# lxa9867/ImageFolder

Hardware: NVIDIA H100
Metric: tokenizer_train_images_per_sec_256x256 (higher is better)
Workload: dtype bf16

## Files before the change

imagefolder_b200/csrc/attn_kernel.cu:

```cuda
#include "xq_common.cuh"
#include "xq_tc.cuh"

namespace xq {
using namespace xqtc;

constexpr int AT_BM = 128;
constexpr int AT_BN = 128;
constexpr int AT_D = 64;
constexpr int AT_NS = 2;
constexpr int AT_TILE = AT_BM * AT_D * 2;
constexpr int AT_THREADS = 288;

struct AttnFwdSmem {
    static constexpr int Q = 0;
    static constexpr int K = AT_TILE;
    static constexpr int V = AT_TILE * (1 + AT_NS);
    static constexpr int BAR = AT_TILE * (1 + 2 * AT_NS);
    static constexpr int BYTES = BAR + 256;
};

__device__ __forceinline__ void named_bar_sync(int id, int nthreads) { asm volatile("bar.sync %0, %1;" ::"r"(id), "r"(nthreads) : "memory"); }

__global__ void __launch_bounds__(AT_THREADS, 1)
attn_fwd_kernel(const __grid_constant__ CUtensorMap tmQKV, __nv_bfloat16 *__restrict__ out, float *__restrict__ lse2, int N, int H,
                int nQ , float c ) {
    extern __shared__ uint8_t smem_raw[];
    uint8_t *base = (uint8_t *)(((uintptr_t)smem_raw + 1023) & ~(uintptr_t)1023);
    uint64_t *bars = (uint64_t *)(base + AttnFwdSmem::BAR);
    uint64_t *q_full = bars + 0;
    uint64_t *k_full = bars + 1;
    uint64_t *k_empty = bars + 1 + AT_NS;
    uint64_t *v_full = bars + 1 + 2 * AT_NS;
    uint64_t *v_empty = bars + 1 + 3 * AT_NS;

    const int tid = threadIdx.x, warp = tid >> 5, lane = tid & 31;
    const int nK = (N + AT_BN - 1) / AT_BN;
    const int bh = blockIdx.x / nQ, qt = blockIdx.x - bh * nQ;
    const int b = bh / H, h = bh - b * H;

    if (tid == 0) {
        mbar_init(q_full, 1);
        for (int i = 0; i < AT_NS; ++i) { mbar_init(&k_full[i], 1); mbar_init(&k_empty[i], 8); mbar_init(&v_full[i], 1); mbar_init(&v_empty[i], 8); }
        mbar_fence_init();
    }
    __syncthreads();

    if (warp == 8) {
        const int colQ = h * AT_D, colK = (H + h) * AT_D, colV = (2 * H + h) * AT_D;
        if (elect_one()) {
            tma_prefetch_desc(&tmQKV);
            mbar_expect_tx(q_full, AT_TILE);
            tma_load_3d(base + AttnFwdSmem::Q, &tmQKV, colQ, qt * AT_BM, b, q_full);
        }
        __syncwarp();
        for (int j = 0; j < nK; ++j) {
            const int st = j % AT_NS;
            const uint32_t ph = ((j / AT_NS) & 1) ^ 1;
            mbar_wait(&k_empty[st], ph);
            if (elect_one()) {
                mbar_expect_tx(&k_full[st], AT_TILE);
                tma_load_3d(base + AttnFwdSmem::K + st * AT_TILE, &tmQKV, colK, j * AT_BN, b, &k_full[st]);
            }
            __syncwarp();
            mbar_wait(&v_empty[st], ph);
            if (elect_one()) {
                mbar_expect_tx(&v_full[st], AT_TILE);
                tma_load_3d(base + AttnFwdSmem::V + st * AT_TILE, &tmQKV, colV, j * AT_BN, b, &v_full[st]);
            }
            __syncwarp();
        }
        return;
    }

    const int wg = warp >> 2, wq = warp & 3;
    const int rq = wg * 64 + wq * 16 + (lane >> 2), cq = 2 * (lane & 3);
    const uint64_t qd = desc_k_sw128(smem_u32(base + AttnFwdSmem::Q + wg * (AT_TILE / 2)));
    float m[2] = {-CUDART_INF_F, -CUDART_INF_F}, l[2] = {0.f, 0.f};
    float o[32];
#pragma unroll
    for (int i = 0; i < 32; ++i) o[i] = 0.f;
    mbar_wait(q_full, 0);
    for (int j = 0; j < nK; ++j) {
        const int st = j % AT_NS;
        const uint32_t ph = (j / AT_NS) & 1;
        float s[64];
        mbar_wait(&k_full[st], ph);
        const uint64_t kd = desc_k_sw128(smem_u32(base + AttnFwdSmem::K + st * AT_TILE));
        wgmma_fence();
#pragma unroll
        for (int k = 0; k < AT_D / 16; ++k) wgmma_m64n128k16_ss<0, 0>(s, desc_adv(qd, k * 32), desc_adv(kd, k * 32), (uint32_t)k);
        wgmma_commit();
        wgmma_wait<0>();
        fence_regs(s);
        __syncwarp();
        if (lane == 0) mbar_arrive(&k_empty[st]);
        const int nv = N - j * AT_BN;
        if (nv < AT_BN) {
#pragma unroll
            for (int i = 0; i < 64; ++i)
                if (8 * (i >> 2) + cq + (i & 1) >= nv) s[i] = -CUDART_INF_F;
        }
        float mx[2] = {m[0], m[1]};
#pragma unroll
        for (int i = 0; i < 64; ++i) mx[(i >> 1) & 1] = fmaxf(mx[(i >> 1) & 1], s[i]);
#pragma unroll
        for (int hh = 0; hh < 2; ++hh) {
            mx[hh] = fmaxf(mx[hh], __shfl_xor_sync(0xffffffffu, mx[hh], 1));
            mx[hh] = fmaxf(mx[hh], __shfl_xor_sync(0xffffffffu, mx[hh], 2));
        }
        float alpha[2], mc[2];
#pragma unroll
        for (int hh = 0; hh < 2; ++hh) {
            alpha[hh] = ex2_approx((m[hh] - mx[hh]) * c);
            m[hh] = mx[hh];
            mc[hh] = mx[hh] * c;
            l[hh] *= alpha[hh];
        }
#pragma unroll
        for (int i = 0; i < 32; ++i) o[i] *= alpha[(i >> 1) & 1];
        uint32_t pa[AT_BN / 16][4];
#pragma unroll
        for (int i = 0; i < 64; i += 2) {
            const int hh = (i >> 1) & 1;
            const float p0 = ex2_approx(fmaf(s[i], c, -mc[hh])), p1 = ex2_approx(fmaf(s[i + 1], c, -mc[hh]));
            l[hh] += p0 + p1;
            pa[i >> 3][((i >> 2) & 1) * 2 + hh] = pack_bf16(p0, p1);
        }
        mbar_wait(&v_full[st], ph);
        const uint64_t vd = desc_mn_sw128(smem_u32(base + AttnFwdSmem::V + st * AT_TILE), AT_TILE);
        wgmma_fence();
#pragma unroll
        for (int k = 0; k < AT_BN / 16; ++k) wgmma_m64n64k16_rs<1>(o, pa[k], desc_adv(vd, k * 2048), 1u);
        wgmma_commit();
        wgmma_wait<0>();
        fence_regs(o);
        __syncwarp();
        if (lane == 0) mbar_arrive(&v_empty[st]);
    }
#pragma unroll
    for (int hh = 0; hh < 2; ++hh) {
        l[hh] += __shfl_xor_sync(0xffffffffu, l[hh], 1);
        l[hh] += __shfl_xor_sync(0xffffffffu, l[hh], 2);
    }
#pragma unroll
    for (int hh = 0; hh < 2; ++hh) {
        const int n = qt * AT_BM + rq + 8 * hh;
        if (n >= N) continue;
        const float inv = 1.0f / l[hh];
        if (cq == 0) lse2[(size_t)bh * N + n] = fmaf(m[hh], c, log2f(l[hh]));
        __nv_bfloat16 *orow = out + ((size_t)b * N + n) * H * AT_D + h * AT_D;
#pragma unroll
        for (int jj = 0; jj < AT_D / 8; ++jj)
            *reinterpret_cast<uint32_t *>(orow + 8 * jj + cq) = pack_bf16(o[4 * jj + 2 * hh] * inv, o[4 * jj + 2 * hh + 1] * inv);
    }
}

constexpr int AT_TAIL_MAX = 0;

__global__ void __launch_bounds__(128)
attn_fwd_tail_kernel(const __nv_bfloat16 *__restrict__ qkv, __nv_bfloat16 *__restrict__ out, float *__restrict__ lse2, int B, int N,
                     int H, int n0 , float c) {
    const int lane = threadIdx.x & 31;
    const long long w = ((long long)blockIdx.x * blockDim.x + threadIdx.x) >> 5;
    const int nt = N - n0;
    if (w >= (long long)B * H * nt) return;
    const int r = (int)(w % nt);
    const int bh = (int)(w / nt);
    const int b = bh / H, h = bh - b * H;
    const int n = n0 + r;
    const size_t W = (size_t)3 * H * AT_D;
    const __nv_bfloat16 *qp = qkv + ((size_t)b * N + n) * W + h * AT_D;
    float qf[AT_D];
#pragma unroll
    for (int u = 0; u < 8; ++u) {
        const uint4 x = *reinterpret_cast<const uint4 *>(qp + u * 8);
        const __nv_bfloat162 *x2 = reinterpret_cast<const __nv_bfloat162 *>(&x);
#pragma unroll
        for (int e = 0; e < 4; ++e) {
            const float2 f = __bfloat1622float2(x2[e]);
            qf[u * 8 + 2 * e] = f.x * c;
            qf[u * 8 + 2 * e + 1] = f.y * c;
        }
    }
    float m = -CUDART_INF_F, l = 0.f, o[AT_D];
#pragma unroll
    for (int i = 0; i < AT_D; ++i) o[i] = 0.f;
    for (int key = lane; key < N; key += 32) {
        const __nv_bfloat16 *kp = qkv + ((size_t)b * N + key) * W + (H + h) * AT_D;
        const __nv_bfloat16 *vp = kp + (size_t)H * AT_D;
        float s = 0.f;
#pragma unroll
        for (int u = 0; u < 8; ++u) {
            const uint4 x = *reinterpret_cast<const uint4 *>(kp + u * 8);
            const __nv_bfloat162 *x2 = reinterpret_cast<const __nv_bfloat162 *>(&x);
#pragma unroll
            for (int e = 0; e < 4; ++e) {
                const float2 f = __bfloat1622float2(x2[e]);
                s = fmaf(qf[u * 8 + 2 * e], f.x, s);
                s = fmaf(qf[u * 8 + 2 * e + 1], f.y, s);
            }
        }
        const float m_new = fmaxf(m, s);
        const float corr = ex2_approx(m - m_new);
        const float p = ex2_approx(s - m_new);
        l = fmaf(l, corr, p);
        m = m_new;
#pragma unroll
        for (int u = 0; u < 8; ++u) {
            const uint4 x = *reinterpret_cast<const uint4 *>(vp + u * 8);
            const __nv_bfloat162 *x2 = reinterpret_cast<const __nv_bfloat162 *>(&x);
#pragma unroll
            for (int e = 0; e < 4; ++e) {
                const float2 f = __bfloat1622float2(x2[e]);
                o[u * 8 + 2 * e] = fmaf(o[u * 8 + 2 * e], corr, p * f.x);
                o[u * 8 + 2 * e + 1] = fmaf(o[u * 8 + 2 * e + 1], corr, p * f.y);
            }
        }
    }
    float M = m;
#pragma unroll
    for (int off = 16; off > 0; off >>= 1) M = fmaxf(M, __shfl_xor_sync(0xffffffffu, M, off));
    const float f = (m == -CUDART_INF_F) ? 0.f : ex2_approx(m - M);
    l *= f;
#pragma unroll
    for (int off = 16; off > 0; off >>= 1) l += __shfl_xor_sync(0xffffffffu, l, off);
    const float inv = 1.0f / l;
    float mine0 = 0.f, mine1 = 0.f;
#pragma unroll
    for (int i = 0; i < AT_D; ++i) {
        float x = o[i] * f;
#pragma unroll
        for (int off = 16; off > 0; off >>= 1) x += __shfl_xor_sync(0xffffffffu, x, off);
        if (i == 2 * lane) mine0 = x;
        if (i == 2 * lane + 1) mine1 = x;
    }
    __nv_bfloat16 *op = out + ((size_t)b * N + n) * H * AT_D + h * AT_D;
    *reinterpret_cast<uint32_t *>(op + 2 * lane) = pack_bf16(mine0 * inv, mine1 * inv);
    if (lane == 0) lse2[(size_t)bh * N + n] = M + log2f(l);
}

constexpr int AB_THREADS = 288;
constexpr int AB_BQ = 64;
constexpr int AB_QS = 3;
constexpr int AB_QTILE = AB_BQ * AT_D * 2;

struct AttnBwdSmem {
    static constexpr int K = 0;
    static constexpr int V = AT_TILE;
    static constexpr int Q = 2 * AT_TILE;
    static constexpr int DO = Q + AB_QS * AB_QTILE;
    static constexpr int DS = DO + AB_QS * AB_QTILE;
    static constexpr int STAT = DS + 2 * AB_QTILE;
    static constexpr int BAR = STAT + AB_QS * 512;
    static constexpr int BYTES = BAR + 256;
};

__device__ __forceinline__ void bwd_epilogue_frag(const float (&acc)[32], float mul, __nv_bfloat16 *__restrict__ row0,
                                                  size_t row_stride, bool ok0, bool ok1, float *__restrict__ g_bias_cols, int lane) {
    const int cq = 2 * (lane & 3);
#pragma unroll
    for (int jj = 0; jj < AT_D / 8; ++jj) {
        const uint32_t w0 = pack_bf16(acc[4 * jj] * mul, acc[4 * jj + 1] * mul);
        const uint32_t w1 = pack_bf16(acc[4 * jj + 2] * mul, acc[4 * jj + 3] * mul);
        if (ok0) *reinterpret_cast<uint32_t *>(row0 + 8 * jj + cq) = w0;
        if (ok1) *reinterpret_cast<uint32_t *>(row0 + 8 * row_stride + 8 * jj + cq) = w1;
        if (g_bias_cols) {
            float s0 = __uint_as_float(w0 << 16) + __uint_as_float(w1 << 16);
            float s1 = __uint_as_float(w0 & 0xffff0000u) + __uint_as_float(w1 & 0xffff0000u);
#pragma unroll
            for (int o = 4; o < 32; o <<= 1) {
                s0 += __shfl_xor_sync(0xffffffffu, s0, o);
                s1 += __shfl_xor_sync(0xffffffffu, s1, o);
            }
            if (lane < 4) {
                atomicAdd(g_bias_cols + 8 * jj + cq, s0);
                atomicAdd(g_bias_cols + 8 * jj + cq + 1, s1);
            }
        }
    }
}

__global__ void __launch_bounds__(AB_THREADS, 1)
attn_bwd_kernel(const __grid_constant__ CUtensorMap tmQKV, const __grid_constant__ CUtensorMap tmDO, const float *__restrict__ lseP,
                const float *__restrict__ deltaP, float *__restrict__ dq_acc, __nv_bfloat16 *__restrict__ dqkv, float *__restrict__ g_bias,
                int N, int H, int Npad, float c, float scale) {
    extern __shared__ uint8_t smem_raw[];
    uint8_t *base = (uint8_t *)(((uintptr_t)smem_raw + 1023) & ~(uintptr_t)1023);
    uint64_t *bars = (uint64_t *)(base + AttnBwdSmem::BAR);
    uint64_t *kv_full = bars;
    uint64_t *q_full = bars + 1;
    uint64_t *q_empty = bars + 1 + AB_QS;
    float *s_lse = (float *)(base + AttnBwdSmem::STAT);
    float *s_delta = s_lse + AB_QS * AB_BQ;

    const int tid = threadIdx.x, warp = tid >> 5, lane = tid & 31;
    const int bh = blockIdx.y, b = bh / H, h = bh - b * H;
    const int k0 = blockIdx.x * AT_BN;
    const int colQ = h * AT_D, colK = (H + h) * AT_D, colV = (2 * H + h) * AT_D;
    const int nQ = (N + AB_BQ - 1) / AB_BQ;

    if (tid == 0) {
        mbar_init(kv_full, 1);
        for (int i = 0; i < AB_QS; ++i) { mbar_init(&q_full[i], 1); mbar_init(&q_empty[i], 8); }
        mbar_fence_init();
    }
    __syncthreads();

    if (warp == 8) {
        if (elect_one()) {
            tma_prefetch_desc(&tmQKV);
            tma_prefetch_desc(&tmDO);
            mbar_expect_tx(kv_full, 2 * AT_TILE);
            for (int hf = 0; hf < 2; ++hf) {
                tma_load_3d(base + AttnBwdSmem::K + hf * AB_QTILE, &tmQKV, colK, k0 + hf * AB_BQ, b, kv_full);
                tma_load_3d(base + AttnBwdSmem::V + hf * AB_QTILE, &tmQKV, colV, k0 + hf * AB_BQ, b, kv_full);
            }
        }
        __syncwarp();
        for (int i = 0; i < nQ; ++i) {
            const int st = i % AB_QS;
            mbar_wait(&q_empty[st], ((i / AB_QS) & 1) ^ 1);
// ... 323 lines not shown

static int attn_bwd_ktail(int N) {
    const int r = N % AT_BN;
    return (N > AT_BN && r != 0 && r <= AB_KTAIL_MAX) ? r : 0;
}

static size_t attn_bwd_ws_layout(int B, int N, int H, size_t *off_lse, size_t *off_delta, size_t *off_dst) {
    const size_t Npad = ((size_t)N + AT_BM - 1) / AT_BM * AT_BM;
    const size_t acc = align_up((size_t)B * H * N * AT_D * sizeof(float), 1024);
    const size_t st = align_up((size_t)B * H * Npad * sizeof(float), 1024);
    const size_t dst = align_up((size_t)B * H * N * attn_bwd_ktail(N) * sizeof(float), 1024);
    if (off_lse) *off_lse = acc;
    if (off_delta) *off_delta = acc + st;
    if (off_dst) *off_dst = acc + 2 * st;
    return acc + 2 * st + dst;
}

}

extern "C" {

size_t xq_vit_attn_bwd_workspace_bytes(int B, int N, int H) {
    if (B <= 0 || N <= 0 || H <= 0) return 0;
    return xq::attn_bwd_ws_layout(B, N, H, nullptr, nullptr, nullptr);
}

int xq_vit_attn_bwd(const void *qkv, const void *out, const void *d_out, const float *lse2, void *dqkv, float *g_bias, int B, int N,
                    int H, int head_dim, float scale, void *workspace, size_t workspace_bytes, void *stream) {
    using namespace xq;
    if (!qkv || !out || !d_out || !lse2 || !dqkv || !workspace || B <= 0 || N <= 0 || H <= 0) return XQ_ERR_ARG;
    if (head_dim != AT_D) return XQ_ERR_UNSUPPORTED;
    if (((uintptr_t)qkv & 15) || ((uintptr_t)out & 15) || ((uintptr_t)d_out & 15) || ((uintptr_t)dqkv & 15) || ((uintptr_t)workspace & 255))
        return XQ_ERR_ARG;
    size_t off_lse, off_delta, off_dst;
    if (workspace_bytes < attn_bwd_ws_layout(B, N, H, &off_lse, &off_delta, &off_dst)) return XQ_ERR_WORKSPACE;
    cudaStream_t st = (cudaStream_t)stream;
    float *acc = (float *)workspace;
    float *lseP = (float *)((char *)workspace + off_lse);
    float *deltaP = (float *)((char *)workspace + off_delta);
    float *dsT = (float *)((char *)workspace + off_dst);
    const uint64_t W = (uint64_t)3 * H * AT_D, Wo = (uint64_t)H * AT_D;
    CUtensorMap tmQKV, tmDO;
    if (!tensor_map_bf16_3d(&tmQKV, qkv, W, N, B, W * 2, (uint64_t)N * W * 2, AB_BQ) ||
        !tensor_map_bf16_3d(&tmDO, d_out, Wo, N, B, Wo * 2, (uint64_t)N * Wo * 2, AB_BQ))
        return XQ_ERR_UNSUPPORTED;
    const int nt = attn_bwd_ktail(N);
    const int nK = nt ? N / AT_BN : (N + AT_BN - 1) / AT_BN;
    const int Npad = (N + AT_BM - 1) / AT_BM * AT_BM;
    if ((long long)B * H > 65535) return XQ_ERR_UNSUPPORTED;
    if (g_bias) XQ_CUDA_TRY(cudaMemsetAsync(g_bias, 0, (size_t)3 * H * AT_D * sizeof(float), st));
    const float c2 = scale * 1.4426950408889634f;
    {
        dim3 grid(nt ? 1u : (unsigned)(Npad / AB_PREP_ROWS), (unsigned)(B * H));
        const size_t ps = nt ? (size_t)2 * 3 * (AB_PREP_ROWS / 32) * 256 * 16 : 0;
        decltype(&attn_bwd_prep_kernel<0>) const preps[] = {attn_bwd_prep_kernel<0>, attn_bwd_prep_kernel<1>, attn_bwd_prep_kernel<2>,
                                                            attn_bwd_prep_kernel<3>, attn_bwd_prep_kernel<4>};
        const auto prep = preps[nt < 4 ? nt : 4];
        if (int rc = smem_optin(prep, ps)) return rc;
        prep<<<grid, 256, ps, st>>>((const __nv_bfloat16 *)qkv, (const __nv_bfloat16 *)out, (const __nv_bfloat16 *)d_out, lse2, lseP,
                                    deltaP, acc, dsT, (__nv_bfloat16 *)dqkv, g_bias, N, H, Npad, c2, scale);
        XQ_LAUNCH_CHECK("attn_bwd_prep_kernel");
    }
    const size_t smem = AttnBwdSmem::BYTES + 1024;
    if (int rc = smem_optin(attn_bwd_kernel, smem)) return rc;
    attn_bwd_kernel<<<dim3((unsigned)nK, (unsigned)(B * H)), AB_THREADS, smem, st>>>(tmQKV, tmDO, lseP, deltaP, acc,
                                                                                     (__nv_bfloat16 *)dqkv, g_bias, N, H, Npad, c2, scale);
    XQ_LAUNCH_CHECK("attn_bwd_kernel");
    {
        dim3 grid((unsigned)((N + AB_CONV_ROWS - 1) / AB_CONV_ROWS), (unsigned)(B * H));
        attn_dq_convert_kernel<<<grid, 256, 0, st>>>(acc, (const __nv_bfloat16 *)qkv, dsT, (__nv_bfloat16 *)dqkv, g_bias, N, H, N - nt, nt, scale);
        XQ_LAUNCH_CHECK("attn_dq_convert_kernel");
    }
    return XQ_OK;
}

int xq_vit_attn_fwd(const void *qkv, void *out, float *lse2, int B, int N, int H, int head_dim, float scale, void *stream) {
    using namespace xq;
    if (!qkv || !out || !lse2 || B <= 0 || N <= 0 || H <= 0) return XQ_ERR_ARG;
    if (head_dim != AT_D) return XQ_ERR_UNSUPPORTED;
    if (((uintptr_t)qkv & 15) || ((uintptr_t)out & 15)) return XQ_ERR_ARG;
    const uint64_t W = (uint64_t)3 * H * AT_D;
    CUtensorMap tmQKV;
    if (!tensor_map_bf16_3d(&tmQKV, qkv, W, N, B, W * 2, (uint64_t)N * W * 2, AT_BM)) return XQ_ERR_UNSUPPORTED;
    const int n_tail = (N % AT_BM != 0 && N % AT_BM <= AT_TAIL_MAX && N > AT_BM) ? N % AT_BM : 0;
    const int nQ = n_tail ? N / AT_BM : (N + AT_BM - 1) / AT_BM;
    const size_t smem = AttnFwdSmem::BYTES + 1024;
    if (int rc = smem_optin(attn_fwd_kernel, smem)) return rc;
    const long long tiles = (long long)B * H * nQ;
    if (tiles > 0x7fffffffLL) return XQ_ERR_ARG;
    const float c = scale * 1.4426950408889634f;
    attn_fwd_kernel<<<(unsigned)tiles, AT_THREADS, smem, (cudaStream_t)stream>>>(tmQKV, (__nv_bfloat16 *)out, lse2, N, H, nQ, c);
    XQ_LAUNCH_CHECK("attn_fwd_kernel");
    if (n_tail) {
        const long long warps = (long long)B * H * n_tail;
        attn_fwd_tail_kernel<<<(unsigned)((warps + 3) / 4), 128, 0, (cudaStream_t)stream>>>(
            (const __nv_bfloat16 *)qkv, (__nv_bfloat16 *)out, lse2, B, N, H, N - n_tail, c);
        XQ_LAUNCH_CHECK("attn_fwd_tail_kernel");
    }
    return XQ_OK;
}

}
```

imagefolder_b200/csrc/xq_tc.cuh:

```cuda
#pragma once
#include <cuda.h>
#include <cuda_bf16.h>
#include <cuda_runtime.h>
#include <stdint.h>

#include <cstring>
#include <mutex>

namespace xqtc {

__device__ __forceinline__ uint32_t smem_u32(const void *p) { return (uint32_t)__cvta_generic_to_shared(p); }

__device__ __forceinline__ void mbar_init(uint64_t *bar, uint32_t count) {
    asm volatile("mbarrier.init.shared::cta.b64 [%0], %1;" ::"r"(smem_u32(bar)), "r"(count));
}
__device__ __forceinline__ void mbar_fence_init() { asm volatile("fence.mbarrier_init.release.cluster;" ::: "memory"); }
__device__ __forceinline__ void mbar_expect_tx(uint64_t *bar, uint32_t bytes) {
    asm volatile("mbarrier.arrive.expect_tx.shared::cta.b64 _, [%0], %1;" ::"r"(smem_u32(bar)), "r"(bytes) : "memory");
}
__device__ __forceinline__ void mbar_arrive(uint64_t *bar) {
    asm volatile("mbarrier.arrive.shared::cta.b64 _, [%0];" ::"r"(smem_u32(bar)) : "memory");
}
__device__ __forceinline__ bool mbar_test(uint64_t *bar, uint32_t parity) {
    uint32_t done;
// ... 12 lines not shown
        "{\n\t.reg .pred p;\n\t"
        "mbarrier.try_wait.parity.shared::cta.b64 p, [%1], %2;\n\t"
        "selp.b32 %0, 1, 0, p;\n\t}"
        : "=r"(done)
        : "r"(smem_u32(bar)), "r"(parity)
        : "memory");
    return done != 0;
}
__device__ __forceinline__ void mbar_wait(uint64_t *bar, uint32_t parity) {
    while (!mbar_try(bar, parity)) {}
}
__device__ __forceinline__ void mbar_wait_ptx(uint64_t *bar, uint32_t parity) {
    asm volatile(
        "{\n\t.reg .pred p;\n\tXQ_MBAR_WAIT:\n\t"
        "mbarrier.try_wait.parity.shared::cta.b64 p, [%0], %1;\n\t"
        "@p bra XQ_MBAR_DONE;\n\tbra XQ_MBAR_WAIT;\n\tXQ_MBAR_DONE:\n\t}" ::"r"(smem_u32(bar)), "r"(parity) : "memory");
}

__device__ __forceinline__ void tma_prefetch_desc(const CUtensorMap *map) {
    asm volatile("prefetch.tensormap [%0];" ::"l"(reinterpret_cast<uint64_t>(map)) : "memory");
}
__device__ __forceinline__ void bulk_g2s(void *dst, const void *src, uint32_t bytes, uint64_t *bar) {
    asm volatile("cp.async.bulk.shared::cluster.global.mbarrier::complete_tx::bytes [%0], [%1], %2, [%3];"
                 ::"r"(smem_u32(dst)), "l"(src), "r"(bytes), "r"(smem_u32(bar))
                 : "memory");
}
__device__ __forceinline__ void tma_load_2d(void *dst, const CUtensorMap *map, int c0, int c1, uint64_t *bar) {
    asm volatile(
        "cp.async.bulk.tensor.2d.shared::cluster.global.mbarrier::complete_tx::bytes [%0], [%1, {%2, %3}], [%4];"
        ::"r"(smem_u32(dst)), "l"(reinterpret_cast<uint64_t>(map)), "r"(c0), "r"(c1), "r"(smem_u32(bar))
        : "memory");
}
__device__ __forceinline__ void tma_load_3d(void *dst, const CUtensorMap *map, int c0, int c1, int c2, uint64_t *bar) {
    asm volatile(
        "cp.async.bulk.tensor.3d.shared::cluster.global.mbarrier::complete_tx::bytes [%0], [%1, {%2, %3, %4}], [%5];"
        ::"r"(smem_u32(dst)), "l"(reinterpret_cast<uint64_t>(map)), "r"(c0), "r"(c1), "r"(c2), "r"(smem_u32(bar))
        : "memory");
}
__device__ __forceinline__ void tma_store_3d(const CUtensorMap *map, const void *src, int c0, int c1, int c2) {
    asm volatile("cp.async.bulk.tensor.3d.global.shared::cta.bulk_group [%0, {%2, %3, %4}], [%1];"
                 ::"l"(reinterpret_cast<uint64_t>(map)), "r"(smem_u32(src)), "r"(c0), "r"(c1), "r"(c2)
                 : "memory");
}
__device__ __forceinline__ void tma_reduce_add_3d(const CUtensorMap *map, const void *src, int c0, int c1, int c2) {
    asm volatile("cp.reduce.async.bulk.tensor.3d.global.shared::cta.add.tile.bulk_group [%0, {%2, %3, %4}], [%1];"
                 ::"l"(reinterpret_cast<uint64_t>(map)), "r"(smem_u32(src)), "r"(c0), "r"(c1), "r"(c2)
                 : "memory");
}
__device__ __forceinline__ void bulk_commit() { asm volatile("cp.async.bulk.commit_group;" ::: "memory"); }
template <int N>
__device__ __forceinline__ void bulk_wait_read() { asm volatile("cp.async.bulk.wait_group.read %0;" ::"n"(N) : "memory"); }
template <int N>
__device__ __forceinline__ void bulk_wait() { asm volatile("cp.async.bulk.wait_group %0;" ::"n"(N) : "memory"); }

__device__ __forceinline__ void fence_async_smem() { asm volatile("fence.proxy.async.shared::cta;" ::: "memory"); }

__device__ __forceinline__ uint64_t desc_k_sw128(uint32_t smem_addr) {
    uint64_t d = 0;
    d |= (uint64_t)((smem_addr & 0x3FFFFu) >> 4);
    d |= (uint64_t)1 << 16;
    d |= (uint64_t)(1024 >> 4) << 32;
    d |= (uint64_t)1 << 62;
    return d;
}
__device__ __forceinline__ uint64_t desc_mn_sw128(uint32_t smem_addr, uint32_t lbo_bytes) {
    uint64_t d = 0;
    d |= (uint64_t)((smem_addr & 0x3FFFFu) >> 4);
    d |= (uint64_t)((lbo_bytes >> 4) & 0x3FFFu) << 16;
    d |= (uint64_t)(1024 >> 4) << 32;
    d |= (uint64_t)1 << 62;
    return d;
}
__device__ __forceinline__ uint64_t desc_adv(uint64_t d, uint32_t bytes) { return d + (uint64_t)(bytes >> 4); }

__device__ __forceinline__ void wgmma_fence() { asm volatile("wgmma.fence.sync.aligned;" ::: "memory"); }
__device__ __forceinline__ void wgmma_commit() { asm volatile("wgmma.commit_group.sync.aligned;" ::: "memory"); }
template <int N>
__device__ __forceinline__ void wgmma_wait() { asm volatile("wgmma.wait_group.sync.aligned %0;" ::"n"(N) : "memory"); }
template <int N>
__device__ __forceinline__ void fence_regs(float (&d)[N]) {
#pragma unroll
    for (int i = 0; i < N; ++i) asm volatile("" : "+f"(d[i])::"memory");
}

template <int TA, int TB>
__device__ __forceinline__ void wgmma_m64n64k16_ss(float (&d)[32], uint64_t da, uint64_t db, uint32_t acc) {
    asm volatile(
        "{\n\t.reg .pred p;\n\tsetp.ne.b32 p, %34, 0;\n\t"
        "wgmma.mma_async.sync.aligned.m64n64k16.f32.bf16.bf16 "
        "{%0, %1, %2, %3, %4, %5, %6, %7, %8, %9, %10, %11, %12, %13, %14, %15, %16, %17, %18, %19, %20, %21, %22, %23, %24, %25, %26, %27, %28, %29, %30, %31}, %32, %33, p, 1, 1, %35, %36;\n\t}"
        : "+f"(d[0]), "+f"(d[1]), "+f"(d[2]), "+f"(d[3]), "+f"(d[4]), "+f"(d[5]), "+f"(d[6]), "+f"(d[7]), "+f"(d[8]), "+f"(d[9]), "+f"(d[10]), "+f"(d[11]), "+f"(d[12]), "+f"(d[13]), "+f"(d[14]), "+f"(d[15]), "+f"(d[16]), "+f"(d[17]), "+f"(d[18]), "+f"(d[19]), "+f"(d[20]), "+f"(d[21]), "+f"(d[22]), "+f"(d[23]), "+f"(d[24]), "+f"(d[25]), "+f"(d[26]), "+f"(d[27]), "+f"(d[28]), "+f"(d[29]), "+f"(d[30]), "+f"(d[31])
        : "l"(da), "l"(db), "r"(acc), "n"(TA), "n"(TB));
}

template <int TA, int TB>
__device__ __forceinline__ void wgmma_m64n128k16_ss(float (&d)[64], uint64_t da, uint64_t db, uint32_t acc) {
    asm volatile(
        "{\n\t.reg .pred p;\n\tsetp.ne.b32 p, %66, 0;\n\t"
        "wgmma.mma_async.sync.aligned.m64n128k16.f32.bf16.bf16 "
        "{%0, %1, %2, %3, %4, %5, %6, %7, %8, %9, %10, %11, %12, %13, %14, %15, %16, %17, %18, %19, %20, %21, %22, %23, %24, %25, %26, %27, %28, %29, %30, %31, %32, %33, %34, %35, %36, %37, %38, %39, %40, %41, %42, %43, %44, %45, %46, %47, %48, %49, %50, %51, %52, %53, %54, %55, %56, %57, %58, %59, %60, %61, %62, %63}, %64, %65, p, 1, 1, %67, %68;\n\t}"
        : "+f"(d[0]), "+f"(d[1]), "+f"(d[2]), "+f"(d[3]), "+f"(d[4]), "+f"(d[5]), "+f"(d[6]), "+f"(d[7]), "+f"(d[8]), "+f"(d[9]), "+f"(d[10]), "+f"(d[11]), "+f"(d[12]), "+f"(d[13]), "+f"(d[14]), "+f"(d[15]), "+f"(d[16]), "+f"(d[17]), "+f"(d[18]), "+f"(d[19]), "+f"(d[20]), "+f"(d[21]), "+f"(d[22]), "+f"(d[23]), "+f"(d[24]), "+f"(d[25]), "+f"(d[26]), "+f"(d[27]), "+f"(d[28]), "+f"(d[29]), "+f"(d[30]), "+f"(d[31]), "+f"(d[32]), "+f"(d[33]), "+f"(d[34]), "+f"(d[35]), "+f"(d[36]), "+f"(d[37]), "+f"(d[38]), "+f"(d[39]), "+f"(d[40]), "+f"(d[41]), "+f"(d[42]), "+f"(d[43]), "+f"(d[44]), "+f"(d[45]), "+f"(d[46]), "+f"(d[47]), "+f"(d[48]), "+f"(d[49]), "+f"(d[50]), "+f"(d[51]), "+f"(d[52]), "+f"(d[53]), "+f"(d[54]), "+f"(d[55]), "+f"(d[56]), "+f"(d[57]), "+f"(d[58]), "+f"(d[59]), "+f"(d[60]), "+f"(d[61]), "+f"(d[62]), "+f"(d[63])
        : "l"(da), "l"(db), "r"(acc), "n"(TA), "n"(TB));
}

template <int TB>
__device__ __forceinline__ void wgmma_m64n64k16_rs(float (&d)[32], const uint32_t (&a)[4], uint64_t db, uint32_t acc) {
    asm volatile(
        "{\n\t.reg .pred p;\n\tsetp.ne.b32 p, %37, 0;\n\t"
        "wgmma.mma_async.sync.aligned.m64n64k16.f32.bf16.bf16 "
        "{%0, %1, %2, %3, %4, %5, %6, %7, %8, %9, %10, %11, %12, %13, %14, %15, %16, %17, %18, %19, %20, %21, %22, %23, %24, %25, %26, %27, %28, %29, %30, %31}, {%32, %33, %34, %35}, %36, p, 1, 1, %38;\n\t}"
        : "+f"(d[0]), "+f"(d[1]), "+f"(d[2]), "+f"(d[3]), "+f"(d[4]), "+f"(d[5]), "+f"(d[6]), "+f"(d[7]), "+f"(d[8]), "+f"(d[9]), "+f"(d[10]), "+f"(d[11]), "+f"(d[12]), "+f"(d[13]), "+f"(d[14]), "+f"(d[15]), "+f"(d[16]), "+f"(d[17]), "+f"(d[18]), "+f"(d[19]), "+f"(d[20]), "+f"(d[21]), "+f"(d[22]), "+f"(d[23]), "+f"(d[24]), "+f"(d[25]), "+f"(d[26]), "+f"(d[27]), "+f"(d[28]), "+f"(d[29]), "+f"(d[30]), "+f"(d[31])
        : "r"(a[0]), "r"(a[1]), "r"(a[2]), "r"(a[3]), "l"(db), "r"(acc), "n"(TB));
}

__device__ __forceinline__ void wgmma_m64n128k8_tf32(float (&d)[64], uint64_t da, uint64_t db, uint32_t acc) {
    asm volatile(
        "{\n\t.reg .pred p;\n\tsetp.ne.b32 p, %66, 0;\n\t"
        "wgmma.mma_async.sync.aligned.m64n128k8.f32.tf32.tf32 "
        "{%0, %1, %2, %3, %4, %5, %6, %7, %8, %9, %10, %11, %12, %13, %14, %15, %16, %17, %18, %19, %20, %21, %22, %23, %24, %25, %26, %27, %28, %29, %30, %31, %32, %33, %34, %35, %36, %37, %38, %39, %40, %41, %42, %43, %44, %45, %46, %47, %48, %49, %50, %51, %52, %53, %54, %55, %56, %57, %58, %59, %60, %61, %62, %63}, %64, %65, p, 1, 1;\n\t}"
        : "+f"(d[0]), "+f"(d[1]), "+f"(d[2]), "+f"(d[3]), "+f"(d[4]), "+f"(d[5]), "+f"(d[6]), "+f"(d[7]), "+f"(d[8]), "+f"(d[9]), "+f"(d[10]), "+f"(d[11]), "+f"(d[12]), "+f"(d[13]), "+f"(d[14]), "+f"(d[15]), "+f"(d[16]), "+f"(d[17]), "+f"(d[18]), "+f"(d[19]), "+f"(d[20]), "+f"(d[21]), "+f"(d[22]), "+f"(d[23]), "+f"(d[24]), "+f"(d[25]), "+f"(d[26]), "+f"(d[27]), "+f"(d[28]), "+f"(d[29]), "+f"(d[30]), "+f"(d[31]), "+f"(d[32]), "+f"(d[33]), "+f"(d[34]), "+f"(d[35]), "+f"(d[36]), "+f"(d[37]), "+f"(d[38]), "+f"(d[39]), "+f"(d[40]), "+f"(d[41]), "+f"(d[42]), "+f"(d[43]), "+f"(d[44]), "+f"(d[45]), "+f"(d[46]), "+f"(d[47]), "+f"(d[48]), "+f"(d[49]), "+f"(d[50]), "+f"(d[51]), "+f"(d[52]), "+f"(d[53]), "+f"(d[54]), "+f"(d[55]), "+f"(d[56]), "+f"(d[57]), "+f"(d[58]), "+f"(d[59]), "+f"(d[60]), "+f"(d[61]), "+f"(d[62]), "+f"(d[63])
        : "l"(da), "l"(db), "r"(acc));
}

__device__ __forceinline__ void sts128(uint32_t saddr, uint4 v) {
    asm volatile("st.shared.v4.b32 [%0], {%1, %2, %3, %4};" ::"r"(saddr), "r"(v.x), "r"(v.y), "r"(v.z), "r"(v.w) : "memory");
}
__device__ __forceinline__ float4 lds128f(uint32_t saddr) {
    float4 v;
    asm volatile("ld.shared.v4.f32 {%0, %1, %2, %3}, [%4];" : "=f"(v.x), "=f"(v.y), "=f"(v.z), "=f"(v.w) : "r"(saddr) : "memory");
    return v;
}

__device__ __forceinline__ bool elect_one() {
    uint32_t pred;
    asm volatile("{\n\t.reg .pred P;\n\telect.sync _|P, 0xffffffff;\n\tselp.b32 %0, 1, 0, P;\n\t}" : "=r"(pred));
    return pred != 0;
}

__host__ __device__ __forceinline__ uint32_t rowtile_off_bf16(int r, int c) {
    return (uint32_t)(r * 128 + ((((c >> 3) ^ (r & 7)) & 7) << 4) + (c & 7) * 2);
}
__host__ __device__ __forceinline__ uint32_t rowtile_unit(int r, int u) { return (uint32_t)(r * 128 + ((u ^ (r & 7)) << 4)); }

__device__ __forceinline__ uint32_t pack_bf16(float lo, float hi) {
    uint32_t r;
    asm("cvt.rn.bf16x2.f32 %0, %1, %2;" : "=r"(r) : "f"(hi), "f"(lo));
    return r;
}
__device__ __forceinline__ float ex2_approx(float x) {
    float y;
    asm("ex2.approx.ftz.f32 %0, %1;" : "=f"(y) : "f"(x));
    return y;
}

constexpr int TMAP_CACHE = 128;

inline bool tensor_map(CUtensorMap *out, const void *base, CUtensorMapDataType dtype, int rank, const cuuint64_t *dims,
                       const cuuint64_t *strides, const cuuint32_t *box, CUtensorMapSwizzle swizzle) {
    typedef CUresult (*Encode)(CUtensorMap *, CUtensorMapDataType, cuuint32_t, void *, const cuuint64_t *, const cuuint64_t *,
                               const cuuint32_t *, const cuuint32_t *, CUtensorMapInterleave, CUtensorMapSwizzle,
                               CUtensorMapL2promotion, CUtensorMapFloatOOBfill);
    struct Entry { uint64_t key[12]; CUtensorMap map; };
    static std::mutex mu;
    static Entry cache[TMAP_CACHE];
    static int n_cached = 0, next = 0;
    static Encode encode = nullptr;
    if (rank < 1 || rank > 3) return false;
    uint64_t key[12] = {(uint64_t)(uintptr_t)base, (uint64_t)dtype, (uint64_t)rank, (uint64_t)swizzle};
    for (int i = 0; i < rank; ++i) { key[4 + i] = dims[i]; key[7 + i] = box[i]; }
    for (int i = 0; i + 1 < rank; ++i) key[10 + i] = strides[i];
    std::lock_guard<std::mutex> g(mu);
    for (int i = 0; i < n_cached; ++i)
        if (memcmp(cache[i].key, key, sizeof(key)) == 0) { *out = cache[i].map; return true; }
    if (!encode) {
        void *p = nullptr;
        cudaDriverEntryPointQueryResult q;
        if (cudaGetDriverEntryPoint("cuTensorMapEncodeTiled", &p, cudaEnableDefault, &q) != cudaSuccess ||
            q != cudaDriverEntryPointSuccess)
            return false;
        encode = (Encode)p;
    }
    const cuuint32_t estr[3] = {1u, 1u, 1u};
    CUtensorMap m;
    if (encode(&m, dtype, (cuuint32_t)rank, const_cast<void *>(base), dims, strides, box, estr, CU_TENSOR_MAP_INTERLEAVE_NONE,
// ... 19 lines not shown
```

Measured before the change: 643.1.

## Make attention forward persistent with overlapped QK/PV wgmma and short tail tile

```diff
diff --git a/imagefolder_b200/csrc/attn_kernel.cu b/imagefolder_b200/csrc/attn_kernel.cu
--- a/imagefolder_b200/csrc/attn_kernel.cu
+++ b/imagefolder_b200/csrc/attn_kernel.cu
@@ -8,235 +8,267 @@
 constexpr int AT_BN = 128;
 constexpr int AT_D = 64;
 constexpr int AT_NS = 2;
+constexpr int AT_QS = 2;
+constexpr int AT_KTAIL = 16;
 constexpr int AT_TILE = AT_BM * AT_D * 2;
 constexpr int AT_THREADS = 288;
 
 struct AttnFwdSmem {
     static constexpr int Q = 0;
-    static constexpr int K = AT_TILE;
-    static constexpr int V = AT_TILE * (1 + AT_NS);
-    static constexpr int BAR = AT_TILE * (1 + 2 * AT_NS);
+    static constexpr int K = AT_TILE * AT_QS;
+    static constexpr int V = K + AT_TILE * AT_NS;
+    static constexpr int BAR = V + AT_TILE * AT_NS;
     static constexpr int BYTES = BAR + 256;
 };
 
 __device__ __forceinline__ void named_bar_sync(int id, int nthreads) { asm volatile("bar.sync %0, %1;" ::"r"(id), "r"(nthreads) : "memory"); }
 
-__global__ void __launch_bounds__(AT_THREADS, 1)
-attn_fwd_kernel(const __grid_constant__ CUtensorMap tmQKV, __nv_bfloat16 *__restrict__ out, float *__restrict__ lse2, int N, int H,
-                int nQ , float c ) {
-    extern __shared__ uint8_t smem_raw[];
-    uint8_t *base = (uint8_t *)(((uintptr_t)smem_raw + 1023) & ~(uintptr_t)1023);
-    uint64_t *bars = (uint64_t *)(base + AttnFwdSmem::BAR);
-    uint64_t *q_full = bars + 0;
-    uint64_t *k_full = bars + 1;
-    uint64_t *k_empty = bars + 1 + AT_NS;
-    uint64_t *v_full = bars + 1 + 2 * AT_NS;
-    uint64_t *v_empty = bars + 1 + 3 * AT_NS;
-
-    const int tid = threadIdx.x, warp = tid >> 5, lane = tid & 31;
-    const int nK = (N + AT_BN - 1) / AT_BN;
-    const int bh = blockIdx.x / nQ, qt = blockIdx.x - bh * nQ;
-    const int b = bh / H, h = bh - b * H;
-
-    if (tid == 0) {
-        mbar_init(q_full, 1);
-        for (int i = 0; i < AT_NS; ++i) { mbar_init(&k_full[i], 1); mbar_init(&k_empty[i], 8); mbar_init(&v_full[i], 1); mbar_init(&v_empty[i], 8); }
-        mbar_fence_init();
-    }
-    __syncthreads();
-
-    if (warp == 8) {
-        const int colQ = h * AT_D, colK = (H + h) * AT_D, colV = (2 * H + h) * AT_D;
-        if (elect_one()) {
-            tma_prefetch_desc(&tmQKV);
-            mbar_expect_tx(q_full, AT_TILE);
-            tma_load_3d(base + AttnFwdSmem::Q, &tmQKV, colQ, qt * AT_BM, b, q_full);
-        }
+struct AttnFwdConsumer {
+    uint8_t *base;
+    uint64_t *k_full, *k_empty, *v_full, *v_empty;
+    uint64_t qd;
+    int r0;
+    int N, cq, lane;
+    float c;
+    float m[2], l[2], o[32];
+    uint32_t pa[AT_BN / 16][4];
+
+    __device__ __forceinline__ int stage(int j) const { return (r0 + j) % AT_NS; }
+    __device__ __forceinline__ uint32_t phase(int j) const { return ((r0 + j) / AT_NS) & 1; }
+    __device__ __forceinline__ uint64_t kdesc(int j) const { return desc_k_sw128(smem_u32(base + AttnFwdSmem::K + stage(j) * AT_TILE)); }
+    __device__ __forceinline__ uint64_t vdesc(int j) const {
+        return desc_mn_sw128(smem_u32(base + AttnFwdSmem::V + stage(j) * AT_TILE), AT_TILE);
+    }
+    __device__ __forceinline__ void release(uint64_t *bar) {
         __syncwarp();
-        for (int j = 0; j < nK; ++j) {
-            const int st = j % AT_NS;
-            const uint32_t ph = ((j / AT_NS) & 1) ^ 1;
-            mbar_wait(&k_empty[st], ph);
-            if (elect_one()) {
-                mbar_expect_tx(&k_full[st], AT_TILE);
-                tma_load_3d(base + AttnFwdSmem::K + st * AT_TILE, &tmQKV, colK, j * AT_BN, b, &k_full[st]);
-            }
-            __syncwarp();
-            mbar_wait(&v_empty[st], ph);
-            if (elect_one()) {
-                mbar_expect_tx(&v_full[st], AT_TILE);
-                tma_load_3d(base + AttnFwdSmem::V + st * AT_TILE, &tmQKV, colV, j * AT_BN, b, &v_full[st]);
-            }
-            __syncwarp();
-        }
-        return;
-    }
-
-    const int wg = warp >> 2, wq = warp & 3;
-    const int rq = wg * 64 + wq * 16 + (lane >> 2), cq = 2 * (lane & 3);
-    const uint64_t qd = desc_k_sw128(smem_u32(base + AttnFwdSmem::Q + wg * (AT_TILE / 2)));
-    float m[2] = {-CUDART_INF_F, -CUDART_INF_F}, l[2] = {0.f, 0.f};
-    float o[32];
-#pragma unroll
-    for (int i = 0; i < 32; ++i) o[i] = 0.f;
-    mbar_wait(q_full, 0);
-    for (int j = 0; j < nK; ++j) {
-        const int st = j % AT_NS;
-        const uint32_t ph = (j / AT_NS) & 1;
-        float s[64];
-        mbar_wait(&k_full[st], ph);
-        const uint64_t kd = desc_k_sw128(smem_u32(base + AttnFwdSmem::K + st * AT_TILE));
-        wgmma_fence();
-#pragma unroll
-        for (int k = 0; k < AT_D / 16; ++k) wgmma_m64n128k16_ss<0, 0>(s, desc_adv(qd, k * 32), desc_adv(kd, k * 32), (uint32_t)k);
-        wgmma_commit();
-        wgmma_wait<0>();
-        fence_regs(s);
-        __syncwarp();
-        if (lane == 0) mbar_arrive(&k_empty[st]);
+        if (lane == 0) mbar_arrive(bar);
+    }
+
+    template <int NS>
+    __device__ __forceinline__ void issue_s(float (&s)[NS], int j) {
+        const uint64_t kd = kdesc(j);
+#pragma unroll
+        for (int k = 0; k < AT_D / 16; ++k) {
+            if constexpr (NS == 64) wgmma_m64n128k16_ss<0, 0>(s, desc_adv(qd, k * 32), desc_adv(kd, k * 32), (uint32_t)k);
+            else wgmma_m64n16k16_ss<0, 0>(s, desc_adv(qd, k * 32), desc_adv(kd, k * 32), (uint32_t)k);
+        }
+    }
+    template <int NS>
+    __device__ __forceinline__ void issue_pv(int j) {
+        const uint64_t vd = vdesc(j);
+#pragma unroll
+        for (int k = 0; k < NS / 8; ++k) wgmma_m64n64k16_rs<1>(o, pa[k], desc_adv(vd, k * 2048), 1u);
+    }
+    template <int NS>
+    __device__ __forceinline__ void softmax(float (&s)[NS], int j, float (&alpha)[2]) {
         const int nv = N - j * AT_BN;
-        if (nv < AT_BN) {
-#pragma unroll
-            for (int i = 0; i < 64; ++i)
+        if (nv < 2 * NS) {
+#pragma unroll
+            for (int i = 0; i < NS; ++i)
                 if (8 * (i >> 2) + cq + (i & 1) >= nv) s[i] = -CUDART_INF_F;
         }
-        float mx[2] = {m[0], m[1]};
-#pragma unroll
-        for (int i = 0; i < 64; ++i) mx[(i >> 1) & 1] = fmaxf(mx[(i >> 1) & 1], s[i]);
+        float mx[2];
+#pragma unroll
+        for (int hh = 0; hh < 2; ++hh) {
+            float t0 = s[2 * hh], t1 = s[2 * hh + 1], t2 = s[4 + 2 * hh], t3 = s[4 + 2 * hh + 1];
+#pragma unroll
+            for (int q = 2; q < NS / 4; q += 2) {
+                t0 = fmaxf(t0, s[4 * q + 2 * hh]);
+                t1 = fmaxf(t1, s[4 * q + 2 * hh + 1]);
+                t2 = fmaxf(t2, s[4 * q + 4 + 2 * hh]);
+                t3 = fmaxf(t3, s[4 * q + 4 + 2 * hh + 1]);
+            }
+            mx[hh] = fmaxf(m[hh], fmaxf(fmaxf(t0, t1), fmaxf(t2, t3)));
+        }
+        float mc[2];
 #pragma unroll
         for (int hh = 0; hh < 2; ++hh) {
             mx[hh] = fmaxf(mx[hh], __shfl_xor_sync(0xffffffffu, mx[hh], 1));
             mx[hh] = fmaxf(mx[hh], __shfl_xor_sync(0xffffffffu, mx[hh], 2));
-        }
-        float alpha[2], mc[2];
-#pragma unroll
-        for (int hh = 0; hh < 2; ++hh) {
             alpha[hh] = ex2_approx((m[hh] - mx[hh]) * c);
             m[hh] = mx[hh];
             mc[hh] = mx[hh] * c;
             l[hh] *= alpha[hh];
         }
 #pragma unroll
+        for (int i = 0; i < NS; i += 2) {
+            const int hh = (i >> 1) & 1;
+            s[i] = ex2_approx(fmaf(s[i], c, -mc[hh]));
+            s[i + 1] = ex2_approx(fmaf(s[i + 1], c, -mc[hh]));
+            l[hh] += s[i] + s[i + 1];
+        }
+    }
+    template <int NS>
+    __device__ __forceinline__ void rescale_and_pack(const float (&s)[NS], const float (&alpha)[2]) {
+#pragma unroll
         for (int i = 0; i < 32; ++i) o[i] *= alpha[(i >> 1) & 1];
-        uint32_t pa[AT_BN / 16][4];
-#pragma unroll
-        for (int i = 0; i < 64; i += 2) {
-            const int hh = (i >> 1) & 1;
-            const float p0 = ex2_approx(fmaf(s[i], c, -mc[hh])), p1 = ex2_approx(fmaf(s[i + 1], c, -mc[hh]));
-            l[hh] += p0 + p1;
-            pa[i >> 3][((i >> 2) & 1) * 2 + hh] = pack_bf16(p0, p1);
-        }
-        mbar_wait(&v_full[st], ph);
-        const uint64_t vd = desc_mn_sw128(smem_u32(base + AttnFwdSmem::V + st * AT_TILE), AT_TILE);
+#pragma unroll
+        for (int i = 0; i < NS; i += 2) pa[i >> 3][((i >> 2) & 1) * 2 + ((i >> 1) & 1)] = pack_bf16(s[i], s[i + 1]);
+    }
+
+    template <int NS>
+    __device__ __forceinline__ void first() {
+        float s[NS], alpha[2];
+        mbar_wait(&k_full[stage(0)], phase(0));
         wgmma_fence();
-#pragma unroll
-        for (int k = 0; k < AT_BN / 16; ++k) wgmma_m64n64k16_rs<1>(o, pa[k], desc_adv(vd, k * 2048), 1u);
+        issue_s(s, 0);
+        wgmma_commit();
+        wgmma_wait<0>();
+        fence_regs(s);
+        release(&k_empty[stage(0)]);
+        softmax(s, 0, alpha);
+        rescale_and_pack(s, alpha);
+    }
+    template <int NS>
+    __device__ __forceinline__ void step(int j) {
+        float s[NS], alpha[2];
+        mbar_wait(&k_full[stage(j)], phase(j));
+        mbar_wait(&v_full[stage(j - 1)], phase(j - 1));
+        fence_regs(o);
+        wgmma_fence();
+        issue_s(s, j);
+        wgmma_commit();
+        issue_pv<64>(j - 1);
+        wgmma_commit();
+        wgmma_wait<1>();
+        fence_regs(s);
+        release(&k_empty[stage(j)]);
+        softmax(s, j, alpha);
+        wgmma_wait<0>();
+        fence_regs(o);
+        fence_regs(pa);
+        release(&v_empty[stage(j - 1)]);
+        rescale_and_pack(s, alpha);
+    }
+    template <int NS>
+    __device__ __forceinline__ void last(int j) {
+        mbar_wait(&v_full[stage(j)], phase(j));
+        fence_regs(o);
+        wgmma_fence();
+        issue_pv<NS>(j);
         wgmma_commit();
         wgmma_wait<0>();
         fence_regs(o);
-        __syncwarp();
-        if (lane == 0) mbar_arrive(&v_empty[st]);
-    }
-#pragma unroll
-    for (int hh = 0; hh < 2; ++hh) {
-        l[hh] += __shfl_xor_sync(0xffffffffu, l[hh], 1);
-        l[hh] += __shfl_xor_sync(0xffffffffu, l[hh], 2);
-    }
-#pragma unroll
-    for (int hh = 0; hh < 2; ++hh) {
-        const int n = qt * AT_BM + rq + 8 * hh;
-        if (n >= N) continue;
-        const float inv = 1.0f / l[hh];
-        if (cq == 0) lse2[(size_t)bh * N + n] = fmaf(m[hh], c, log2f(l[hh]));
-        __nv_bfloat16 *orow = out + ((size_t)b * N + n) * H * AT_D + h * AT_D;
-#pragma unroll
-        for (int jj = 0; jj < AT_D / 8; ++jj)
-            *reinterpret_cast<uint32_t *>(orow + 8 * jj + cq) = pack_bf16(o[4 * jj + 2 * hh] * inv, o[4 * jj + 2 * hh + 1] * inv);
-    }
-}
-
-constexpr int AT_TAIL_MAX = 0;
-
-__global__ void __launch_bounds__(128)
-attn_fwd_tail_kernel(const __nv_bfloat16 *__restrict__ qkv, __nv_bfloat16 *__restrict__ out, float *__restrict__ lse2, int B, int N,
-                     int H, int n0 , float c) {
-    const int lane = threadIdx.x & 31;
-    const long long w = ((long long)blockIdx.x * blockDim.x + threadIdx.x) >> 5;
-    const int nt = N - n0;
-    if (w >= (long long)B * H * nt) return;
-    const int r = (int)(w % nt);
-    const int bh = (int)(w / nt);
-    const int b = bh / H, h = bh - b * H;
-    const int n = n0 + r;
-    const size_t W = (size_t)3 * H * AT_D;
-    const __nv_bfloat16 *qp = qkv + ((size_t)b * N + n) * W + h * AT_D;
-    float qf[AT_D];
-#pragma unroll
-    for (int u = 0; u < 8; ++u) {
-        const uint4 x = *reinterpret_cast<const uint4 *>(qp + u * 8);
-        const __nv_bfloat162 *x2 = reinterpret_cast<const __nv_bfloat162 *>(&x);
-#pragma unroll
-        for (int e = 0; e < 4; ++e) {
-            const float2 f = __bfloat1622float2(x2[e]);
-            qf[u * 8 + 2 * e] = f.x * c;
-            qf[u * 8 + 2 * e + 1] = f.y * c;
-        }
-    }
-    float m = -CUDART_INF_F, l = 0.f, o[AT_D];
-#pragma unroll
-    for (int i = 0; i < AT_D; ++i) o[i] = 0.f;
-    for (int key = lane; key < N; key += 32) {
-        const __nv_bfloat16 *kp = qkv + ((size_t)b * N + key) * W + (H + h) * AT_D;
-        const __nv_bfloat16 *vp = kp + (size_t)H * AT_D;
-        float s = 0.f;
-#pragma unroll
-        for (int u = 0; u < 8; ++u) {
-            const uint4 x = *reinterpret_cast<const uint4 *>(kp + u * 8);
-            const __nv_bfloat162 *x2 = reinterpret_cast<const __nv_bfloat162 *>(&x);
-#pragma unroll
-            for (int e = 0; e < 4; ++e) {
-                const float2 f = __bfloat1622float2(x2[e]);
-                s = fmaf(qf[u * 8 + 2 * e], f.x, s);
-                s = fmaf(qf[u * 8 + 2 * e + 1], f.y, s);
-            }
-        }
-        const float m_new = fmaxf(m, s);
-        const float corr = ex2_approx(m - m_new);
-        const float p = ex2_approx(s - m_new);
-        l = fmaf(l, corr, p);
-        m = m_new;
-#pragma unroll
-        for (int u = 0; u < 8; ++u) {
-            const uint4 x = *reinterpret_cast<const uint4 *>(vp + u * 8);
-            const __nv_bfloat162 *x2 = reinterpret_cast<const __nv_bfloat162 *>(&x);
-#pragma unroll
-            for (int e = 0; e < 4; ++e) {
-                const float2 f = __bfloat1622float2(x2[e]);
-                o[u * 8 + 2 * e] = fmaf(o[u * 8 + 2 * e], corr, p * f.x);
-                o[u * 8 + 2 * e + 1] = fmaf(o[u * 8 + 2 * e + 1], corr, p * f.y);
-            }
-        }
-    }
-    float M = m;
-#pragma unroll
-    for (int off = 16; off > 0; off >>= 1) M = fmaxf(M, __shfl_xor_sync(0xffffffffu, M, off));
-    const float f = (m == -CUDART_INF_F) ? 0.f : ex2_approx(m - M);
-    l *= f;
-#pragma unroll
-    for (int off = 16; off > 0; off >>= 1) l += __shfl_xor_sync(0xffffffffu, l, off);
-    const float inv = 1.0f / l;
-    float mine0 = 0.f, mine1 = 0.f;
-#pragma unroll
-    for (int i = 0; i < AT_D; ++i) {
-        float x = o[i] * f;
-#pragma unroll
-        for (int off = 16; off > 0; off >>= 1) x += __shfl_xor_sync(0xffffffffu, x, off);
-        if (i == 2 * lane) mine0 = x;
-        if (i == 2 * lane + 1) mine1 = x;
-    }
-    __nv_bfloat16 *op = out + ((size_t)b * N + n) * H * AT_D + h * AT_D;
-    *reinterpret_cast<uint32_t *>(op + 2 * lane) = pack_bf16(mine0 * inv, mine1 * inv);
-    if (lane == 0) lse2[(size_t)bh * N + n] = M + log2f(l);
+        fence_regs(pa);
+        release(&v_empty[stage(j)]);
+    }
+    __device__ __forceinline__ void skip(int nK) {
+        for (int j = 0; j < nK; ++j) {
+            mbar_wait(&k_full[stage(j)], phase(j));
+            release(&k_empty[stage(j)]);
+            mbar_wait(&v_full[stage(j)], phase(j));
+            release(&v_empty[stage(j)]);
+        }
+    }
+};
+
+__global__ void __launch_bounds__(AT_THREADS, 1)
+attn_fwd_kernel(const __grid_constant__ CUtensorMap tmQKV, __nv_bfloat16 *__restrict__ out, float *__restrict__ lse2, int N, int H,
+                int nQ , int tiles , float c ) {
+    extern __shared__ uint8_t smem_raw[];
+    uint8_t *base = (uint8_t *)(((uintptr_t)smem_raw + 1023) & ~(uintptr_t)1023);
+    uint64_t *bars = (uint64_t *)(base + AttnFwdSmem::BAR);
+    uint64_t *q_full = bars;
+    uint64_t *q_empty = bars + AT_QS;
+    uint64_t *k_full = bars + 2 * AT_QS;
+    uint64_t *k_empty = k_full + AT_NS;
+    uint64_t *v_full = k_full + 2 * AT_NS;
+    uint64_t *v_empty = k_full + 3 * AT_NS;
+
+    const int tid = threadIdx.x, warp = tid >> 5, lane = tid & 31;
+    const int nK = (N + AT_BN - 1) / AT_BN;
+
+    if (tid == 0) {
+        for (int i = 0; i < AT_QS; ++i) { mbar_init(&q_full[i], 1); mbar_init(&q_empty[i], 8); }
+        for (int i = 0; i < AT_NS; ++i) { mbar_init(&k_full[i], 1); mbar_init(&k_empty[i], 8); mbar_init(&v_full[i], 1); mbar_init(&v_empty[i], 8); }
+        mbar_fence_init();
+    }
+    __syncthreads();
+
+    if (warp == 8) {
+        if (elect_one()) tma_prefetch_desc(&tmQKV);
+        int r = 0;
+        for (int t = blockIdx.x, ti = 0; t < tiles; t += gridDim.x, ++ti) {
+            const int bh = t / nQ, qt = t - bh * nQ;
+            const int b = bh / H, h = bh - b * H;
+            const int colQ = h * AT_D, colK = (H + h) * AT_D, colV = (2 * H + h) * AT_D;
+            const int qs = ti % AT_QS;
+            mbar_wait(&q_empty[qs], ((ti / AT_QS) & 1) ^ 1);
+            if (elect_one()) {
+                mbar_expect_tx(&q_full[qs], AT_TILE);
+                tma_load_3d(base + AttnFwdSmem::Q + qs * AT_TILE, &tmQKV, colQ, qt * AT_BM, b, &q_full[qs]);
+            }
+            __syncwarp();
+            for (int j = 0; j < nK; ++j, ++r) {
+                const int st = r % AT_NS;
+                const uint32_t ph = ((r / AT_NS) & 1) ^ 1;
+                mbar_wait(&k_empty[st], ph);
+                if (elect_one()) {
+                    mbar_expect_tx(&k_full[st], AT_TILE);
+                    tma_load_3d(base + AttnFwdSmem::K + st * AT_TILE, &tmQKV, colK, j * AT_BN, b, &k_full[st]);
+                }
+                __syncwarp();
+                mbar_wait(&v_empty[st], ph);
+                if (elect_one()) {
+                    mbar_expect_tx(&v_full[st], AT_TILE);
+                    tma_load_3d(base + AttnFwdSmem::V + st * AT_TILE, &tmQKV, colV, j * AT_BN, b, &v_full[st]);
+                }
+                __syncwarp();
+            }
+        }
+        return;
+    }
+
+    const int wg = warp >> 2, wq = warp & 3;
+    const int rq = wg * 64 + wq * 16 + (lane >> 2), cq = 2 * (lane & 3);
+    const bool short_last = N - (nK - 1) * AT_BN <= AT_KTAIL;
+    AttnFwdConsumer cs;
+    cs.base = base;
+    cs.k_full = k_full; cs.k_empty = k_empty; cs.v_full = v_full; cs.v_empty = v_empty;
+    cs.N = N; cs.cq = cq; cs.lane = lane; cs.c = c;
+    cs.r0 = 0;
+    for (int t = blockIdx.x, ti = 0; t < tiles; t += gridDim.x, ++ti, cs.r0 += nK) {
+        const int bh = t / nQ, qt = t - bh * nQ;
+        const int b = bh / H, h = bh - b * H;
+        const int qs = ti % AT_QS;
+        if (qt * AT_BM + wg * 64 >= N) {
+            cs.skip(nK);
+            cs.release(&q_empty[qs]);
+            continue;
+        }
+        cs.qd = desc_k_sw128(smem_u32(base + AttnFwdSmem::Q + qs * AT_TILE + wg * (AT_TILE / 2)));
+        cs.m[0] = cs.m[1] = -CUDART_INF_F;
+        cs.l[0] = cs.l[1] = 0.f;
+#pragma unroll
+        for (int i = 0; i < 32; ++i) cs.o[i] = 0.f;
+        mbar_wait(&q_full[qs], (ti / AT_QS) & 1);
+        if (nK == 1 && short_last) cs.first<8>();
+        else cs.first<64>();
+        for (int j = 1; j < nK; ++j) {
+            if (j == nK - 1 && short_last) cs.step<8>(j);
+            else cs.step<64>(j);
+        }
+        if (short_last) cs.last<8>(nK - 1);
+        else cs.last<64>(nK - 1);
+        cs.release(&q_empty[qs]);
+        float *l = cs.l;
+#pragma unroll
+        for (int hh = 0; hh < 2; ++hh) {
+            l[hh] += __shfl_xor_sync(0xffffffffu, l[hh], 1);
+            l[hh] += __shfl_xor_sync(0xffffffffu, l[hh], 2);
+        }
+#pragma unroll
+        for (int hh = 0; hh < 2; ++hh) {
+            const int n = qt * AT_BM + rq + 8 * hh;
+            if (n >= N) continue;
+            const float inv = 1.0f / l[hh];
+            if (cq == 0) lse2[(size_t)bh * N + n] = fmaf(cs.m[hh], c, log2f(l[hh]));
+            __nv_bfloat16 *orow = out + ((size_t)b * N + n) * H * AT_D + h * AT_D;
+#pragma unroll
+            for (int jj = 0; jj < AT_D / 8; ++jj)
+                *reinterpret_cast<uint32_t *>(orow + 8 * jj + cq) = pack_bf16(cs.o[4 * jj + 2 * hh] * inv, cs.o[4 * jj + 2 * hh + 1] * inv);
+        }
+    }
 }
 
 constexpr int AB_THREADS = 288;
@@ -726,21 +758,17 @@
     const uint64_t W = (uint64_t)3 * H * AT_D;
     CUtensorMap tmQKV;
     if (!tensor_map_bf16_3d(&tmQKV, qkv, W, N, B, W * 2, (uint64_t)N * W * 2, AT_BM)) return XQ_ERR_UNSUPPORTED;
-    const int n_tail = (N % AT_BM != 0 && N % AT_BM <= AT_TAIL_MAX && N > AT_BM) ? N % AT_BM : 0;
-    const int nQ = n_tail ? N / AT_BM : (N + AT_BM - 1) / AT_BM;
+    const int nQ = (N + AT_BM - 1) / AT_BM;
     const size_t smem = AttnFwdSmem::BYTES + 1024;
     if (int rc = smem_optin(attn_fwd_kernel, smem)) return rc;
+    int sms = 0;
+    if (int rc = sm_count(&sms)) return rc;
     const long long tiles = (long long)B * H * nQ;
-    if (tiles > 0x7fffffffLL) return XQ_ERR_ARG;
+    if (tiles + sms > 0x7fffffffLL) return XQ_ERR_ARG;
+    const int grid = (int)(tiles < sms ? tiles : sms);
     const float c = scale * 1.4426950408889634f;
-    attn_fwd_kernel<<<(unsigned)tiles, AT_THREADS, smem, (cudaStream_t)stream>>>(tmQKV, (__nv_bfloat16 *)out, lse2, N, H, nQ, c);
+    attn_fwd_kernel<<<grid, AT_THREADS, smem, (cudaStream_t)stream>>>(tmQKV, (__nv_bfloat16 *)out, lse2, N, H, nQ, (int)tiles, c);
     XQ_LAUNCH_CHECK("attn_fwd_kernel");
-    if (n_tail) {
-        const long long warps = (long long)B * H * n_tail;
-        attn_fwd_tail_kernel<<<(unsigned)((warps + 3) / 4), 128, 0, (cudaStream_t)stream>>>(
-            (const __nv_bfloat16 *)qkv, (__nv_bfloat16 *)out, lse2, B, N, H, N - n_tail, c);
-        XQ_LAUNCH_CHECK("attn_fwd_tail_kernel");
-    }
     return XQ_OK;
 }
 
diff --git a/imagefolder_b200/csrc/xq_tc.cuh b/imagefolder_b200/csrc/xq_tc.cuh
--- a/imagefolder_b200/csrc/xq_tc.cuh
+++ b/imagefolder_b200/csrc/xq_tc.cuh
@@ -118,6 +118,13 @@
 #pragma unroll
     for (int i = 0; i < N; ++i) asm volatile("" : "+f"(d[i])::"memory");
 }
+template <int N>
+__device__ __forceinline__ void fence_regs(uint32_t (&a)[N][4]) {
+#pragma unroll
+    for (int i = 0; i < N; ++i)
+#pragma unroll
+        for (int e = 0; e < 4; ++e) asm volatile("" : "+r"(a[i][e])::"memory");
+}
 
 template <int TA, int TB>
 __device__ __forceinline__ void wgmma_m64n64k16_ss(float (&d)[32], uint64_t da, uint64_t db, uint32_t acc) {
@@ -136,6 +143,16 @@
         "wgmma.mma_async.sync.aligned.m64n128k16.f32.bf16.bf16 "
         "{%0, %1, %2, %3, %4, %5, %6, %7, %8, %9, %10, %11, %12, %13, %14, %15, %16, %17, %18, %19, %20, %21, %22, %23, %24, %25, %26, %27, %28, %29, %30, %31, %32, %33, %34, %35, %36, %37, %38, %39, %40, %41, %42, %43, %44, %45, %46, %47, %48, %49, %50, %51, %52, %53, %54, %55, %56, %57, %58, %59, %60, %61, %62, %63}, %64, %65, p, 1, 1, %67, %68;\n\t}"
         : "+f"(d[0]), "+f"(d[1]), "+f"(d[2]), "+f"(d[3]), "+f"(d[4]), "+f"(d[5]), "+f"(d[6]), "+f"(d[7]), "+f"(d[8]), "+f"(d[9]), "+f"(d[10]), "+f"(d[11]), "+f"(d[12]), "+f"(d[13]), "+f"(d[14]), "+f"(d[15]), "+f"(d[16]), "+f"(d[17]), "+f"(d[18]), "+f"(d[19]), "+f"(d[20]), "+f"(d[21]), "+f"(d[22]), "+f"(d[23]), "+f"(d[24]), "+f"(d[25]), "+f"(d[26]), "+f"(d[27]), "+f"(d[28]), "+f"(d[29]), "+f"(d[30]), "+f"(d[31]), "+f"(d[32]), "+f"(d[33]), "+f"(d[34]), "+f"(d[35]), "+f"(d[36]), "+f"(d[37]), "+f"(d[38]), "+f"(d[39]), "+f"(d[40]), "+f"(d[41]), "+f"(d[42]), "+f"(d[43]), "+f"(d[44]), "+f"(d[45]), "+f"(d[46]), "+f"(d[47]), "+f"(d[48]), "+f"(d[49]), "+f"(d[50]), "+f"(d[51]), "+f"(d[52]), "+f"(d[53]), "+f"(d[54]), "+f"(d[55]), "+f"(d[56]), "+f"(d[57]), "+f"(d[58]), "+f"(d[59]), "+f"(d[60]), "+f"(d[61]), "+f"(d[62]), "+f"(d[63])
+        : "l"(da), "l"(db), "r"(acc), "n"(TA), "n"(TB));
+}
+
+template <int TA, int TB>
+__device__ __forceinline__ void wgmma_m64n16k16_ss(float (&d)[8], uint64_t da, uint64_t db, uint32_t acc) {
+    asm volatile(
+        "{\n\t.reg .pred p;\n\tsetp.ne.b32 p, %10, 0;\n\t"
+        "wgmma.mma_async.sync.aligned.m64n16k16.f32.bf16.bf16 "
+        "{%0, %1, %2, %3, %4, %5, %6, %7}, %8, %9, p, 1, 1, %11, %12;\n\t}"
+        : "+f"(d[0]), "+f"(d[1]), "+f"(d[2]), "+f"(d[3]), "+f"(d[4]), "+f"(d[5]), "+f"(d[6]), "+f"(d[7])
         : "l"(da), "l"(db), "r"(acc), "n"(TA), "n"(TB));
 }
 
```

Result: faster. 652.7 (median of 6 runs) (+1.5%).
